# victorca25/traiNNer

Hardware: AMD Instinct MI355X
Metric: HR images/sec (G+D step), ESRGAN x4 128->512 (higher is better)
Workload: dtype f32 (bf16x3)

## Files before the change

### trainner_amd/csrc/conv_sweep.hip

```cpp
#include <stddef.h>
#include <string.h>
#include <type_traits>
#include <utility>
#include "conv_body.h"
#include "conv_epilogue.h"
#include "conv_handoff.h"

namespace {

constexpr int SW_TH = 8, SW_TW = 32, SW_HT = SW_TH + 2, SW_WT = SW_TW + 2;
constexpr int SW_ROW = TNR_X3_ROW;
constexpr int SW_A_ROWS = SW_HT * SW_WT;
constexpr int SW_A_ALLOC_ROWS = 384;
constexpr int SW_A_FLOATS = SW_A_ALLOC_ROWS * SW_ROW;
constexpr int SW_UNIT_FLOATS = 32 * SW_ROW;
constexpr int SW_SLOT_UNITS = 9;
constexpr int SW_SLOT_FLOATS = SW_SLOT_UNITS * SW_UNIT_FLOATS;
constexpr int SW_RING = 3;
constexpr size_t SW_LDS_BYTES = (size_t)(2 * SW_A_FLOATS + SW_RING * SW_SLOT_FLOATS) * sizeof(float);
constexpr int SW_NPASS = 9, SW_NSTAGE = 5, SW_NTILE = 6;
constexpr int SW_A_IT = (SW_A_ROWS * 4 + 511) / 512;
constexpr int SW_B_PIECES = (SW_SLOT_UNITS * 3 + 7) / 8;
static_assert(SW_LDS_BYTES <= 160 * 1024, "one sweep workgroup per CU");

// ... 8 lines not shown
__host__ __device__ constexpr int sw_nj_rt(int p) { return p == 7 ? 1 : ((p == 0 || p == 1 || p == 3) ? 3 : 2); }
__host__ __device__ constexpr int sw_j0_rt(int p) { return p == 0 ? 0 : (p == 2 ? 1 : (p == 4 ? 2 : (p == 5 || p == 8 ? 4 : (p == 7 ? 5 : 3)))); }
__host__ __device__ constexpr int sw_T_rt(int p) { return p == 7 ? 9 : 3; }
constexpr bool sw_plan_ok() {
    for (int p = 0; p < SW_NPASS; ++p) {
        if (SW_TT[p] * SW_NJ[p] > SW_SLOT_UNITS || 9 % SW_TT[p]) return false;
        if (sw_nj_rt(p) != SW_NJ[p] || sw_j0_rt(p) != SW_J0[p] || sw_T_rt(p) != SW_TT[p]) return false;
        if (sw_apass(p) && SW_J0[p] != (sw_phase(p) < 4 ? sw_phase(p) : 4)) return false;
        if (!sw_apass(p) && SW_J0[p] != SW_J0[p - 1] + SW_NJ[p - 1]) return false;
        if ((!sw_apass(p) || p == 8) && SW_J0[p] + SW_NJ[p] != SW_NTILE) return false;
    }
    return true;
}

static_assert(sw_plan_ok(), "sweep plan");
static_assert(SW_J0[1] == SW_J0[3] && SW_NJ[1] == SW_NJ[3] && SW_TT[1] == SW_TT[3] && SW_J0[5] == SW_J0[8] && SW_NJ[5] == SW_NJ[8] && SW_TT[5] == SW_TT[8], "passes 1 / 3 and 5 / 8 share a body");

struct SweepK {
    int nck0;
    int tiles_x, tiles_y, tpi, tiles;
    unsigned *progress;
    unsigned base;
    unsigned *err;
    int nxcd;
    unsigned *disp;
    const float *wq;
    int wq_bytes;
    ConvK st[SW_NSTAGE];
};

__host__ __device__ inline int sw_nchunks(int p, int nck0) { return sw_phase(p) == 0 ? nck0 : 2; }
__host__ __device__ inline int sw_ch_lo(int p, int nck0) { return sw_phase(p) == 0 ? 0 : 16 * nck0 + 32 * (sw_phase(p) - 1); }
__host__ __device__ inline int sw_total_units(int nck0) {
    int u = 0;
    for (int p = 0; p < SW_NPASS; ++p) u += sw_nchunks(p, nck0) * 9 * sw_nj_rt(p);
    return u;
}

struct SweepPackK {
    int nck0, units;
    int direct;
    const float *wp[SW_NSTAGE];
    int KinP[SW_NSTAGE], KoutP[SW_NSTAGE];
    float *out;
};

__device__ __forceinline__ void sweep_pack_one(const SweepPackK &a, const int g) {
    const int unit = g >> 6, r = (g >> 1) & 31, sp = g & 1;
    if (unit >= a.units) return;
    int p = 0, u0 = 0;
    for (; p < SW_NPASS; ++p) {
        const int n = sw_nchunks(p, a.nck0) * 9 * sw_nj_rt(p);
        if (unit < u0 + n) break;
        u0 += n;
    }
    const int lu = unit - u0, nj = sw_nj_rt(p);
    const int jj = lu % nj, ct = lu / nj, tap = ct % 9, ck = ct / 9;
    const int j = sw_j0_rt(p) + jj;
    const int s = j < 4 ? j : 4, cb = j == 5 ? 1 : 0;
    const int h = sp ^ ((r >> TNR_X3_SWZ) & 1);
    const int ch = sw_ch_lo(p, a.nck0) + 16 * ck + 8 * h;
    const float *src = a.wp[s] + ((size_t)tap * a.KoutP[s] + cb * 32 + r) * a.KinP[s] + ch;
    const f32x4 q0 = *reinterpret_cast<const f32x4 *>(src), q1 = *reinterpret_cast<const f32x4 *>(src + 4);
    tnr_bf16x8 pl[3];
    tnr_split_bf16x3(q0, q1, pl);
    if (a.direct) {
        float *dst = a.out + (size_t)unit * SW_UNIT_FLOATS + (h * 32 + r) * 4;
#pragma unroll
        for (int k = 0; k < 3; ++k) *reinterpret_cast<tnr_bf16x8 *>(dst + k * 256) = pl[k];
        return;
    }
    float *dst = a.out + (size_t)unit * SW_UNIT_FLOATS + r * SW_ROW + 4 * sp;
#pragma unroll
// ... 305 lines not shown
}

constexpr int S4_A_IT = (SW_A_ROWS * 4 + 255) / 256;
constexpr int S4_PIECES = (SW_SLOT_UNITS * 3 + 3) / 4;
static_assert(S4_PIECES <= 8 && S4_A_IT == 6, "the DMA / side-work plan: 8 DMA steps behind a synchronisation, 6 items per chunk");

template <int B, class F, int... I>
__device__ __forceinline__ void sw_static_for_seq(F &f, std::integer_sequence<int, I...>) {
    (f(std::integral_constant<int, B + I>{}), ...);
}
template <int B, int E, class F>
__device__ __forceinline__ void sw_static_for(F &&f) {
    sw_static_for_seq<B>(f, std::make_integer_sequence<int, (E > B ? E - B : 0)>{});
}

template <int J0, int NJ, bool DIRECT, class Sync, class Item, class Dma, class Tick, class BFetch>
__device__ __forceinline__ void sweep4_chunk(f32x16 (&acc)[2][SW_NTILE], const float *sa, const float *s_b_lane, const int (&apix0)[2],
                                             const int half, Sync &&sync, Item &&item_step, Dma &&dma_step, Tick &&tick,
                                             tnr_bf16x8 (&fbr)[3][3], BFetch &&b_fetch) {
    static_assert((9 * NJ) % 3 == 0, "a chunk starts at ring position 0");
    constexpr int TA[6] = {0, 2, 1, 0, 1, 0}, TB[6] = {2, 0, 1, 1, 0, 0};
    constexpr int NU = 9 * NJ, SU = 3 * NJ;
    tnr_bf16x8 fa[2][2][3], fb[2][3];
    const float *a_src[2][2];
    auto addr_a = [&](auto tc) __attribute__((always_inline)) {
        constexpr int t = decltype(tc)::value, dy = t / 3, dx = t % 3;
#pragma unroll
        for (int m = 0; m < 2; ++m) {
            const int pp = apix0[m] + dy * SW_WT + dx;
            a_src[t & 1][m] = sa + pp * SW_ROW + 4 * (half ^ ((pp >> TNR_X3_SWZ) & 1));
        }
    };
    auto read_a = [&](auto tc, int m, int sp) __attribute__((always_inline)) {
        constexpr int t = decltype(tc)::value;
        fa[t & 1][m][sp] = *reinterpret_cast<const tnr_bf16x8 *>(a_src[t & 1][m] + 8 * sp);
// ... 38 lines not shown
            }
            if constexpr (NEXT_TAP && i >= 3 && i < 9) read_a(std::integral_constant<int, (t + 1 < 9 ? t + 1 : 8)>{}, (i - 3) / 3, (i - 3) % 3);
            if constexpr (DMA_UNIT && i % S4_DMA_EVERY == S4_DMA_EVERY - 1) dma_step();
            if constexpr (ITEM >= 0 && ITEM < S4_A_IT && i >= 4 && i < 9) item_step(std::integral_constant<int, (ITEM >= 0 && ITEM < S4_A_IT ? ITEM : 0)>{}, std::integral_constant<int, (i >= 4 && i < 9 ? i - 4 : 0)>{});
            __builtin_amdgcn_sched_barrier(0);
        });
#ifdef SW_TIMELINE
        if constexpr (NJ == 3 || NJ == 2) {
            constexpr int cls = SYNC_UNIT ? 0 : ((u % SU) <= 1 ? 1 : (ITEM >= 0 && ITEM < S4_A_IT ? 2 : 3));
            tick(cls + (NJ == 2 ? 4 : 0), __builtin_amdgcn_s_memtime() - tu0);
        }
#endif
    });
}

template <int J0, int NJ, class Item, class BFetch>
__device__ __forceinline__ void amp4_chunk(f32x16 (&acc)[2][SW_NTILE], const float *sa, const int (&apix0)[2], const int half,
                                           Item &&item, tnr_bf16x8 (&fbq)[9], BFetch &&b_fetch) {
    constexpr int NU = 9 * NJ;
    static_assert(NU % 9 == 0, "a chunk starts at ring position 0");
    tnr_bf16x8 fa[2][2];
    const float *a_src[2][2];
    auto addr_a = [&](auto tc) __attribute__((always_inline)) {
        constexpr int t = decltype(tc)::value, dy = t / 3, dx = t % 3;
#pragma unroll
        for (int m = 0; m < 2; ++m) {
            const int pp = apix0[m] + dy * SW_WT + dx;
            a_src[t & 1][m] = sa + pp * SW_ROW + 4 * (half ^ ((pp >> TNR_X3_SWZ) & 1));
        }
    };
    addr_a(std::integral_constant<int, 0>{});
    fa[0][0] = *reinterpret_cast<const tnr_bf16x8 *>(a_src[0][0]);
// ... 9 lines not shown
        if constexpr (NEXT_TAP) fa[(t + 1) & 1][0] = *reinterpret_cast<const tnr_bf16x8 *>(a_src[(t + 1) & 1][0]);
        __builtin_amdgcn_sched_barrier(0);
        acc[1][J0 + jj] = __builtin_amdgcn_mfma_f32_32x32x16_bf16(fa[t & 1][1], fbq[u % 9], acc[1][J0 + jj], 0, 0, 0);
        if constexpr (NEXT_TAP) fa[(t + 1) & 1][1] = *reinterpret_cast<const tnr_bf16x8 *>(a_src[(t + 1) & 1][1]);
        if constexpr (ITEM >= 0 && ITEM < S4_A_IT) item(std::integral_constant<int, (ITEM >= 0 && ITEM < S4_A_IT ? ITEM : 0)>{});
        __builtin_amdgcn_sched_barrier(0);
    });
}

#ifndef S4D_EPI_AFTER
#define S4D_EPI_AFTER 1
#endif
#ifndef S4D_ALOAD_ALWAYS
#define S4D_ALOAD_ALWAYS 1
#endif
template <bool DIRECT, bool AMP = false>
__global__ void __launch_bounds__(256, 1) conv_sweep4_kernel(const SweepK c) {
    static_assert(DIRECT || !AMP, "the bf16-operand form exists as a direct form only");
    extern __shared__ __attribute__((aligned(16))) float smem[];
    float *s_a = smem, *s_b = smem + 2 * SW_A_FLOATS;
    const int tid = threadIdx.x;
    const int wave = __builtin_amdgcn_readfirstlane(tid >> 6), lane = tid & 63, li = lane & 31, half = lane >> 5;
    const int g = gridDim.x;
    const bool xcd_split = (g & 7) == 0 && c.nxcd == 8;
    const int xcd = xcd_split ? ((int)blockIdx.x & 7) : 0, per_x = xcd_split ? (g >> 3) : g;
    __shared__ int s_next_tile;
    auto next_tile = [&]() __attribute__((always_inline)) {
        if (tid == 0) {
            const int slot = (int)atomicAdd(c.disp + xcd, 1u);
            const int kk = slot / per_x, ii = slot - kk * per_x;
            s_next_tile = xcd * per_x + ii + g * kk;
        }
        __syncthreads();
// ... 92 lines not shown
                const int q = wave + 4 * i;
                if (q < pieces) __builtin_amdgcn_raw_ptr_buffer_load_lds(w_rs, dst + q * 256, 16, lane * 16, src0 + q * 1024, 0, 0);
            }
        };
        auto cur_advance = [&](SweepCur &cu) __attribute__((always_inline)) {
            cu.unit += 3 * sw_nj_rt(cu.p);
            if (++cu.sl == 3) {
                cu.sl = 0;
                if (++cu.ck == sw_nchunks(cu.p, c.nck0)) {
                    cu.ck = 0;
                    ++cu.p;
                }
            }
        };

        f32x16 acc[2][SW_NTILE];
#pragma unroll
        for (int m = 0; m < 2; ++m)
#pragma unroll
            for (int j = 0; j < SW_NTILE; ++j)
#pragma unroll
                for (int r = 0; r < 16; ++r) acc[m][j][r] = 0.f;

        SweepCur ld{0, 0, 0, 0};
        a_load(0);
        __syncthreads();
        tnr_bf16x8 fbr[3][3];
        int bq = 0;
        auto b_fetch = [&](auto rc, int sp) __attribute__((always_inline)) {
            constexpr int r = decltype(rc)::value;
            fbr[r][sp] = __builtin_bit_cast(tnr_bf16x8, __builtin_amdgcn_raw_buffer_load_b128(w_rs, lane * 16, (bq * 3 + sp) * 1024, 0));
            if (sp == 2) ++bq;
        };
        tnr_bf16x8 fbq[9];
        auto b_fetch1 = [&](auto rc) __attribute__((always_inline)) {
// ... 97 lines not shown
                conv_epilogue_dpp<TNR_CONV_3x3, SW_TW, 2, 2, true, 8>(a, t, 0, n, ty0, tx0, 0, wave, li, half, y_rs);
            }
            pend_tile = tile;
            pend_value = c.base + (unsigned)S + 1u;
            pend_age = 0;
            { SW_T(t_e1); SW_ADD(8, t_e1 - t_e0); }
        };
        auto sync = [&](auto sc) __attribute__((always_inline)) {
            constexpr int sl = decltype(sc)::value;
            slot_sync((sl + 1) % SW_RING);
        };
        auto item_step = [&](auto ic, auto kc) __attribute__((always_inline)) {
            if (has_next) item_step_buf(ic, kc, (e + 1) & 1);
        };

        sw_static_for<0, SW_NPASS>([&](auto pc) __attribute__((always_inline)) {
            constexpr int p = decltype(pc)::value;
            const int nchunks = sw_nchunks(p, c.nck0), ch_lo = sw_ch_lo(p, c.nck0);
#pragma unroll 1
            for (int ck = 0; ck < nchunks; ++ck) {
                slot_sync(1);
                if constexpr (!sw_apass(p) && !(DIRECT && S4D_EPI_AFTER)) {
                    if (ck == 0) epilogue_of(std::integral_constant<int, sw_phase(p)>{});
                }
                const bool last_ck = ck + 1 == nchunks;
                has_next = !(last_ck && p == SW_NPASS - 1);
                int ch_keep = 0;
                if (has_next) {
                    int ch_next = ch_lo + 16 * (ck + 1);
                    if (last_ck) {
                        ch_next = sw_ch_lo(p + 1 < SW_NPASS ? p + 1 : p, c.nck0);
                        if constexpr (p + 1 < SW_NPASS && sw_apass(p + 1)) {
                            const ChainWait w{c.progress, c.base + (unsigned)sw_phase(p + 1), n, ty, tx, c.tiles_x, c.tiles_y, c.err,
                                              &pend_tile, pend_value};
                            SW_T(t_w0);
                            w();
                            { SW_T(t_w1); SW_ADD(1, t_w1 - t_w0); }
                        }
                    }
                    if constexpr (!(DIRECT && S4D_ALOAD_ALWAYS)) {
                        SW_T(t_al0);
                        a_load(ch_next);
                        { SW_T(t_al1); SW_ADD(2, t_al1 - t_al0); }
                    } else {
                        ch_keep = ch_next;
                    }
                }
                if constexpr (DIRECT && S4D_ALOAD_ALWAYS) {
                    SW_T(t_al0);
                    a_load(ch_keep, has_next);
                    { SW_T(t_al1); SW_ADD(2, t_al1 - t_al0); }
                }
                const float *sa = s_a + (e & 1) * SW_A_FLOATS;
                SW_T(t_c0);
                if constexpr (AMP) {
                    auto item1 = [&](auto ic) __attribute__((always_inline)) {
                        if (has_next) a_item1(ic, (e + 1) & 1);
                    };
                    amp4_chunk<sw_j0(p), sw_nj(p)>(acc, sa, apix0, half, item1, fbq, b_fetch1);
                } else {
                    sweep4_chunk<sw_j0(p), sw_nj(p), DIRECT>(acc, sa, s_b_lane, apix0, half, sync, item_step, dma_step, tick, fbr, b_fetch);
                }
                { SW_T(t_c1); SW_ADD(6, t_c1 - t_c0); SW_ADD(15, 1ull); SW_ADD(9 + (sw_nj(p) == 3 ? 0 : (sw_nj(p) == 2 ? 1 : 2)), t_c1 - t_c0); }
                ++e;
            }
            if constexpr (DIRECT && S4D_EPI_AFTER && sw_apass(p) && p + 1 < SW_NPASS) {
                epilogue_of(std::integral_constant<int, sw_phase(p)>{});
            }
        });
        epilogue_of(std::integral_constant<int, 4>{});
    }
    asm volatile("s_waitcnt vmcnt(0)" ::: "memory");
    __syncthreads();
    if (pend_tile >= 0 && tid == 0) __hip_atomic_store(c.progress + pend_tile, pend_value, __ATOMIC_RELAXED, __HIP_MEMORY_SCOPE_AGENT);
    if (tid == 0 && atomicAdd(c.disp + 8, 1u) == (unsigned)g - 1u) {
#pragma unroll
        for (int i = 0; i < 9; ++i) __hip_atomic_store(c.disp + i, 0u, __ATOMIC_RELAXED, __HIP_MEMORY_SCOPE_AGENT);
    }
#ifdef SW_TIMELINE
    if (tid == 0) {
        tl[14] = __builtin_amdgcn_s_memtime() - tl_begin;
        for (int i = 0; i < 16; ++i) atomicAdd(&sw_tl[i], tl[i]);
        for (int i = 0; i < 16; ++i) atomicAdd(&sw_tl2[i], tl2[i]);
    }
#endif
// ... 416 lines not shown

bool d4_ok(const tnr_conv_desc *d) {
    if (d->shuffle != 0 && !(d->shuffle == 2 && (d->Cout % 256) == 0 && d->r1.ptr == nullptr && d->r2.ptr == nullptr && d->m.ptr == nullptr &&
                             d->noise_pos == 0 && d->pad_mode == 0 && (d->y.ctot % 4) == 0 &&
                             (int64_t)d->N * d->H * d->W * 4 * d->y.ctot < (1LL << 30)))
        return false;
    return d->mode == TNR_CONV_3x3 && (d->mma == TNR_MMA_BF16X3 || d->mma == TNR_MMA_BF16) && (d->pad_mode == 0 || (d->pad_mode == 1 && d->H >= 2 && d->W >= 2)) &&
           (d->Cout % 64) == 0 && d->KoutP == d->Cout &&
           d->Cin == d->KinP && (d->Cin % 16) == 0 && d->Cin >= 32 && d->Ho == d->H && d->Wo == d->W && d->W >= 32 && d->H >= 8 &&
           (int64_t)d->N * d->H * d->W * d->x.ctot < (1LL << 30) && (int64_t)d->N * d->H * d->W * d->y.ctot < (1LL << 30) &&
           (int64_t)(d->Cout / 64) * (d->Cin / 16) * 18 * SW_UNIT_FLOATS * (int64_t)sizeof(float) < (1LL << 31);
}

bool sweep_pattern(const tnr_conv_desc *st, int n, const char **why) {
    auto no = [&](const char *w) { if (why) *why = w; return false; };
    if (n != SW_NSTAGE) return no("not 5 stages");
    const tnr_conv_desc &d0 = st[0];
    if (d0.Cin < 32 || (d0.Cin % 16) != 0) return no("block input channels must be a multiple of 16, >= 32");
    for (int i = 0; i < n; ++i) {
        const tnr_conv_desc &d = st[i];
        if (d.mode != TNR_CONV_3x3 || (d.mma != TNR_MMA_BF16X3 && d.mma != TNR_MMA_BF16) || d.mma != d0.mma || d.pad_mode != 0)
            return no("stage is not a zero-padded 3x3 in bf16x3 (or all stages with bf16 operands)");
        if (d.N != d0.N || d.H != d0.H || d.W != d0.W || d.Ho != d0.H || d.Wo != d0.W) return no("pixel grids differ");
        if (d.x.ptr != d0.x.ptr || d.x.ctot != d0.x.ctot || d.x.coff != d0.x.coff) return no("stages read different buffers");
        if (d.Cin != d0.Cin + 32 * i || d.KinP != d.Cin) return no("input channels do not grow by 32 per stage");
        if (d.Cout != (i < 4 ? 32 : 64) || d.KoutP != d.Cout) return no("output channels are not 32, 32, 32, 32, 64");
        if (i < 4 && (d.y.ptr != d0.x.ptr || d.y.ctot != d0.x.ctot || d.y.coff != d0.x.coff + d.Cin)) return no("stage output is not the next channel group");
        if ((d.x.ctot % 4) || (d.x.coff % 4) || (d.y.ctot % 4) || (d.y.coff % 4)) return no("views must be 4-channel aligned");
        if (d.r1.ptr && ((d.r1.ctot % 4) || (d.r1.coff % 4) || (d.r1_ch % 4))) return no("r1 view");
        if (d.r2.ptr && ((d.r2.ctot % 4) || (d.r2.coff % 4))) return no("r2 view");
        if (d.m.ptr && ((d.m.ctot % 4) || (d.m.coff % 4) || (d.m_lo % 4) || (d.m_hi % 4))) return no("mask view");
        if (d.noise_pos < 0 || d.noise_pos > 2 || (i < 4 && d.noise_pos != 0)) return no("the noise multiplier belongs to the last stage");
        if ((int64_t)d.N * d.H * d.W * d.x.ctot >= (1LL << 30) || (int64_t)d.N * d.H * d.W * d.y.ctot >= (1LL << 30)) return no("buffer above 4 GiB");
        if (!d.x.ptr || !d.y.ptr || !d.wp) return no("null pointer");
    }
    const tnr_conv_desc &dl = st[n - 1];
    if (dl.y.ptr == d0.x.ptr && dl.y.coff < d0.x.coff + dl.Cin && dl.y.coff + dl.Cout > d0.x.coff) return no("last stage overwrites its own input");
    return true;
}

int sweep_form() {
    static const int form = [] {
        const char *w = getenv("TNR_SWEEP_WAVES"), *f = getenv("TNR_SWEEP_FORM");
        if (w && atoi(w) == 8) return 8;
        return (f && f[0] == 'd' && f[1] == 'm') ? 4 : 5;
    }();
    return form;
}
constexpr size_t S4D_LDS_BYTES = (size_t)(2 * SW_A_FLOATS) * sizeof(float);

int sweep_cus() {
    static int cus = 0;
    if (cus == 0) {
        int dev = 0;
        if (hipGetDevice(&dev) != hipSuccess || hipDeviceGetAttribute(&cus, hipDeviceAttributeMultiprocessorCount, dev) != hipSuccess ||
            hipFuncSetAttribute(reinterpret_cast<const void *>(conv_sweep_kernel), hipFuncAttributeMaxDynamicSharedMemorySize,
                                (int)SW_LDS_BYTES) != hipSuccess ||
            hipFuncSetAttribute(reinterpret_cast<const void *>(conv_sweep4_kernel<false>), hipFuncAttributeMaxDynamicSharedMemorySize,
                                (int)SW_LDS_BYTES) != hipSuccess ||
            hipFuncSetAttribute(reinterpret_cast<const void *>(conv_sweep4_kernel<true>), hipFuncAttributeMaxDynamicSharedMemorySize,
                                (int)S4D_LDS_BYTES) != hipSuccess ||
            hipFuncSetAttribute(reinterpret_cast<const void *>(conv_sweep4_kernel<true, true>), hipFuncAttributeMaxDynamicSharedMemorySize,
                                (int)S4D_LDS_BYTES) != hipSuccess || cus < 1)
            cus = -1;
    }
    return cus;
}

}

#ifdef SW_TIMELINE
extern "C" int tnr_debug_sweep_units(unsigned long long *out16, int reset) {
    if (out16 != nullptr && hipMemcpyFromSymbol(out16, HIP_SYMBOL(sw_tl2), sizeof(sw_tl2)) != hipSuccess) return TNR_ELAUNCH;
    if (reset) {
        unsigned long long z[16] = {0, 0, 0, 0, 0, 0, 0, 0, 0, 0, 0, 0, 0, 0, 0, 0};
        if (hipMemcpyToSymbol(HIP_SYMBOL(sw_tl2), z, sizeof(z)) != hipSuccess) return TNR_ELAUNCH;
    }
    return TNR_OK;
}
extern "C" int tnr_debug_sweep_timeline(unsigned long long *out16, int reset) {
    if (out16 != nullptr && hipMemcpyFromSymbol(out16, HIP_SYMBOL(sw_tl), sizeof(sw_tl)) != hipSuccess) return TNR_ELAUNCH;
    if (reset) {
        unsigned long long z[16] = {0, 0, 0, 0, 0, 0, 0, 0, 0, 0, 0, 0, 0, 0, 0, 0};
        if (hipMemcpyToSymbol(HIP_SYMBOL(sw_tl), z, sizeof(z)) != hipSuccess) return TNR_ELAUNCH;
    }
    return TNR_OK;
}
#endif

extern "C" int64_t tnr_conv_sweep_image_bytes(const tnr_conv_desc *stages, int32_t n) {
    if (stages == nullptr || !sweep_pattern(stages, n, nullptr)) return 0;
    if (stages[0].mma == TNR_MMA_BF16 && sweep_form() != 5) return 0;
    const int cus = sweep_cus();
    const int tpi = tnr_cdiv(stages[0].W, SW_TW) * tnr_cdiv(stages[0].H, SW_TH);
    if (cus < 1 || tpi > cus) return 0;
    return (int64_t)sw_total_units(stages[0].Cin / 16) * SW_UNIT_FLOATS * (int64_t)sizeof(float);
}

extern "C" int tnr_conv_sweep_pack(const tnr_conv_desc *stages, int32_t n, void *image, int64_t image_bytes, void *stream) {
    const char *why = "";
    TNR_REQUIRE(stages != nullptr && image != nullptr && sweep_pattern(stages, n, &why), "conv_sweep_pack: not a sweepable dense block (%s)", why);
    SweepPackK a;
    a.nck0 = stages[0].Cin / 16;
    a.units = sw_total_units(a.nck0);
    a.direct = sweep_form() == 5;
    TNR_REQUIRE((int64_t)a.units * SW_UNIT_FLOATS * (int64_t)sizeof(float) <= image_bytes, "conv_sweep_pack: image buffer too small");
    for (int i = 0; i < SW_NSTAGE; ++i) {
        a.wp[i] = stages[i].wp;
        a.KinP[i] = stages[i].KinP;
        a.KoutP[i] = stages[i].KoutP;
    }
    a.out = static_cast<float *>(image);
    hipLaunchKernelGGL(sweep_pack_kernel, dim3((unsigned)tnr_cdiv(a.units * 64, 256)), dim3(256), 0, (hipStream_t)stream, a);
    return tnr_check_launch("conv_sweep_pack");
}

static_assert(sizeof(SweepPackK) <= sizeof(((tnr_sweep_pack_item *)nullptr)->opaque), "tnr_sweep_pack_item holds the pack kernel's arguments");

extern "C" int tnr_conv_sweep_pack_item(const tnr_conv_desc *stages, int32_t n, void *image, int64_t image_bytes, tnr_sweep_pack_item *item) {
    const char *why = "";
    TNR_REQUIRE(stages != nullptr && image != nullptr && item != nullptr && sweep_pattern(stages, n, &why),
                "conv_sweep_pack_item: not a sweepable dense block (%s)", why);
    SweepPackK a;
    a.nck0 = stages[0].Cin / 16;
    a.units = sw_total_units(a.nck0);
    a.direct = sweep_form() == 5;
    TNR_REQUIRE((int64_t)a.units * SW_UNIT_FLOATS * (int64_t)sizeof(float) <= image_bytes, "conv_sweep_pack_item: image buffer too small");
    for (int i = 0; i < SW_NSTAGE; ++i) {
        a.wp[i] = stages[i].wp;
        a.KinP[i] = stages[i].KinP;
        a.KoutP[i] = stages[i].KoutP;
    }
    a.out = static_cast<float *>(image);
    memset(item, 0, sizeof(*item));
    memcpy(item->opaque, &a, sizeof(a));
    item->units = a.units;
    return TNR_OK;
}

extern "C" int tnr_conv_sweep_pack_batch(const tnr_sweep_pack_item *items_dev, int32_t n, int32_t max_units, void *stream) {
    TNR_REQUIRE(items_dev != nullptr && n >= 1 && n <= 65535 && max_units >= 1, "conv_sweep_pack_batch: bad arguments");
    static_assert(sizeof(tnr_sweep_pack_item) % 8 == 0, "table stride");
    hipLaunchKernelGGL(sweep_pack_batch_strided_kernel, dim3((unsigned)tnr_cdiv(max_units * 64, 256), (unsigned)n), dim3(256), 0, (hipStream_t)stream, items_dev);
    return tnr_check_launch("conv_sweep_pack_batch");
}

// ... 8 lines not shown
    TNR_REQUIRE(cus >= 1, "conv_sweep: cannot set up the kernel");
    SweepK c;
    c.nck0 = d0.Cin / 16;
    c.tiles_x = tnr_cdiv(d0.W, SW_TW);
    c.tiles_y = tnr_cdiv(d0.H, SW_TH);
    c.tpi = c.tiles_x * c.tiles_y;
    c.tiles = c.tpi * d0.N;
    TNR_REQUIRE(c.tpi <= cus, "conv_sweep: the %d tiles of an image exceed the %d co-resident workgroups", c.tpi, cus);
    c.progress = ws;
    c.err = tnr_fault_word_or(ws + ws_bytes / 4 - 1);
    static const int nxcd = [] { const char *e = getenv("TNR_SWEEP_DISPENSERS"); return e ? atoi(e) : 1; }();
    c.nxcd = nxcd == 1 ? 1 : 8;
    c.disp = ws + (ws_bytes / 4 - 1 - 4 - CH_CU_KEYS - CH_SWEEP_WORDS);
    c.base = epoch * (uint32_t)(TNR_CHAIN_MAX + 2);
    c.wq = static_cast<const float *>(image);
    c.wq_bytes = sw_total_units(c.nck0) * SW_UNIT_FLOATS * (int)sizeof(float);
    for (int i = 0; i < SW_NSTAGE; ++i) {
        const tnr_conv_desc *d = &stages[i];
        ConvK &k = c.st[i];
        k.x = d->x.ptr; k.x_ct = d->x.ctot; k.x_co = d->x.coff;
        k.N = d->N; k.H = d->H; k.W = d->W; k.Cin = d->Cin;
        k.wp = d->wp; k.KinP = d->KinP; k.KoutP = d->KoutP;
        k.y = d->y.ptr; k.y_ct = d->y.ctot; k.y_co = d->y.coff; k.Ho = d->Ho; k.Wo = d->Wo; k.Cout = d->Cout;
        k.bias = d->bias; k.act = d->act; k.slope = d->slope; k.alpha = d->alpha;
        k.r1 = d->r1.ptr; k.r1_ct = d->r1.ctot; k.r1_co = d->r1.coff; k.r1_ch = d->r1_ch; k.beta1 = d->beta1;
        k.r2 = d->r2.ptr; k.r2_ct = d->r2.ctot; k.r2_co = d->r2.coff; k.alpha2 = d->alpha2;
        k.m = d->m.ptr; k.m_ct = d->m.ctot; k.m_co = d->m.coff; k.m_lo = d->m_lo; k.m_hi = d->m_hi; k.m_slope = d->m_slope;
        k.noise_pos = d->noise_pos; k.noise_sigma = d->noise_sigma; k.noise_k0 = d->noise_key0; k.noise_k1 = d->noise_key1; k.noise_pix0 = d->noise_pix0;
        k.tiles_x = c.tiles_x; k.tiles_y = c.tiles_y; k.ncb = d->KoutP / 32;
        k.th_space = d->Ho; k.tw_space = d->Wo;
        k.ksplit = 1; k.split_stride = 0; k.bf = d->mma; k.reflect = 0;
    }
    const int per_round = (cus / c.tpi) * c.tpi;
    const int grid = c.tiles < per_round ? c.tiles : per_round;
    const int form = sweep_form();
    if (stages[0].mma == TNR_MMA_BF16) {
        TNR_REQUIRE(form == 5, "conv_sweep: bf16 operands (use_amp) run in the direct four-wave form only");
        hipLaunchKernelGGL((conv_sweep4_kernel<true, true>), dim3((unsigned)grid), dim3(256), S4D_LDS_BYTES, (hipStream_t)stream, c);
        return tnr_check_launch("conv_sweep");
    }
    if (form == 8) hipLaunchKernelGGL(conv_sweep_kernel, dim3((unsigned)grid), dim3(512), SW_LDS_BYTES, (hipStream_t)stream, c);
    else if (form == 4) hipLaunchKernelGGL(conv_sweep4_kernel<false>, dim3((unsigned)grid), dim3(256), SW_LDS_BYTES, (hipStream_t)stream, c);
    else hipLaunchKernelGGL(conv_sweep4_kernel<true>, dim3((unsigned)grid), dim3(256), S4D_LDS_BYTES, (hipStream_t)stream, c);
    return tnr_check_launch("conv_sweep");
}

extern "C" int64_t tnr_conv_wq_bytes(const tnr_conv_desc *d) {
    if (d != nullptr && s2_ok(d)) return (int64_t)(d->Cout / 64) * (d->Cin / 16) * 4 * S2_NU * SW_UNIT_FLOATS * (int64_t)sizeof(float);
    if (d == nullptr || !d4_ok(d)) return 0;
    return (int64_t)(d->Cout / 64) * (d->Cin / 16) * 18 * SW_UNIT_FLOATS * (int64_t)sizeof(float);
// ... 129 lines not shown
```

### trainner_amd/models/modules/architectures/RRDBNet_arch.py

```python
import math

import torch
import torch.nn as nn

from .... import ops
from ....engine import ConvOp, HipNet
from ....ops import View, new_act
from . import block as B


class ResidualDenseBlock_5C(nn.Module):
    def __init__(self, nf=64, gc=32, act_type="leakyrelu"):
        super().__init__()
        self.conv1 = B.conv_block(nf, gc, 3, act_type=act_type)
        self.conv2 = B.conv_block(nf + gc, gc, 3, act_type=act_type)
        self.conv3 = B.conv_block(nf + 2 * gc, gc, 3, act_type=act_type)
        self.conv4 = B.conv_block(nf + 3 * gc, gc, 3, act_type=act_type)
        self.conv5 = B.conv_block(nf + 4 * gc, nf, 3, act_type=None)


class RRDB(nn.Module):
    def __init__(self, nf, gc=32, act_type="leakyrelu"):
        super().__init__()
        self.RDB1 = ResidualDenseBlock_5C(nf, gc, act_type)
# ... 78 lines not shown
        for i in range(nrdb):
            buf = bufs[i % nbuf]
            convs = o["rdb"][i]
            st = []
            for k in range(4):
                cin = nf + gc * k
                st.append(convs[k].fwd_stage(View(buf, 0, cin), View(buf, cin, gc), fresh_from=(cin - gc if k else None),
                                             act=act, slope=sl))
            dst = View(bufs[(i + 1) % nbuf], 0, nf) if i + 1 < nrdb else View(trunk)
            nk = dict(noise=nz[i]) if nz else {}
            if i % 3 == 2:
                st.append(convs[4].fwd_stage(View(buf), dst, fresh_from=nf + 3 * gc, alpha=0.2, r1=View(buf, 0, nf),
                                             r2=View(bufs[(i - 2) % nbuf], 0, nf), alpha2=0.2, **nk))
            else:
                st.append(convs[4].fwd_stage(View(buf), dst, fresh_from=nf + 3 * gc, alpha=0.2, r1=View(buf, 0, nf), **nk))
            ops.conv_chain(st)
        y0 = new_act(N, h, w, nf, dev)
        o["lr"].fwd(View(trunk), View(y0), r1=fea_keep)
        cur, stages = View(y0), []
        for u in o["up"]:
            H2, W2 = cur.H * 2, cur.W * 2
            if self.upsample_mode == "upconv":
                nxt = View(new_act(N, H2, W2, nf, dev))
                u.fwd(cur, nxt, act=act, slope=sl)
                stages.append((cur, nxt, None))
            else:
                nxt = View(new_act(N, H2, W2, nf, dev))
                t = None
                if not u.fwd_shuffle2(cur, nxt, act=act, slope=sl):
                    t = View(new_act(N, cur.H, cur.W, 4 * nf, dev))
                    u.fwd(cur, t, act=act, slope=sl)
# ... 38 lines not shown

    def _rdb_backward(self, convs, dense, buf, GP, s, gnext, extra, want_w, pend, nz_out=None):
        nf, gc, sl = self.nf, self.gc, self.slope
        dp = self._dense_packer
        st = []
        for t in range(4):
            cin = nf + t * gc
            xk = View(buf, nf + (3 - t) * gc, gc)
            st.append(dict(x=View(GP, 0, cin), wp=dp.get(dense[t]), y=View(GP, cin, gc), fresh_from=(cin - gc if t else None),
                           mask=xk, m_lo=0, m_hi=gc, m_slope=sl))
        g = View(GP, 0, nf)
        kw = dict(r2=extra, alpha2=1.0) if extra is not None else {}
        if nz_out is not None:
            kw["noise"] = nz_out.at(2)
        st.append(dict(x=View(GP), wp=dp.get(dense[4]), y=gnext, fresh_from=nf + 3 * gc, r1=g, beta1=s, **kw))
        ops.conv_chain(st)
        if want_w:
            pend.setdefault("c5", []).append(convs[4].wgrad_item(View(buf), g, alpha=0.2 * s))
            if ops.WGRAD_PAIR and gc == 32 and nf == 64:
                for ka, kb in ((3, 2), (1, 0)):
                    cin = nf + gc * kb
                    gpair = View(GP, nf + (3 - ka) * gc, 2 * gc)
                    it = convs[ka].wgrad_item(View(buf, 0, cin), gpair)
                    it["pair"] = (convs[kb].mod.weight.grad, None if it["db"] is None else convs[kb].mod.bias.grad, gc)
                    pend["c5"].append(it)
                    ga = View(GP, nf + (3 - ka) * gc, gc)
                    pend.setdefault(gc, []).append(convs[ka].wgrad_item(View(buf, cin, gc), ga, cin_begin=cin))
                return
            for k in (3, 2, 1, 0):
                cin = nf + gc * k
                gk = View(GP, nf + (3 - k) * gc, gc)
# ... 106 lines not shown
```

### trainner_amd/ops.py

```python
import ctypes as C

import os

import torch

from . import hip
from .hip import (ACT_LRELU, ACT_NONE, ACT_RELU, CONV_1x1, CONV_3x3, CONV_3x3_C4, CONV_3x3_UP2, CONV_4x4_S2, CONV_7x7_C4, DGRAD_4x4_S2,
                  PACK_C4_DGRAD3, PACK_C4_FWD, PACK_COL_DGRAD3, PACK_COL_FWD, PACK_DENSE_DGRAD, PACK_DGRAD_3x3, PACK_DGRAD_S2, PACK_FWD, PACK_FWD_S2D, CView,
                  ConvDesc,
                  DensePackItem, PackItem, WgradDesc)


def round_up(a, b):
    return (a + b - 1) // b * b


class View:
    __slots__ = ("buf", "coff", "C")

    def __init__(self, buf, coff=0, C=None):
        assert buf.dim() == 4 and buf.dtype == torch.float32 and buf.is_contiguous()
        self.buf, self.coff = buf, coff
        self.C = buf.shape[3] - coff if C is None else C
        assert 0 <= coff and coff + self.C <= buf.shape[3]
# ... 120 lines not shown
    def add_block(self, weights, nf, gc, scale5):
        lib = hip.load()
        idx = []
        for t in range(5):
            ko, ki, n = hip.c_i(), hip.c_i(), hip.c_l()
            hip.check(lib.tnr_pack_dense_dims(nf, gc, t, C.byref(ko), C.byref(ki), C.byref(n)), "pack_dense_dims")
            self.jobs.append((list(weights), t, nf, gc, float(scale5), ko.value, ki.value, n.value))
            self.packed.append(None)
            idx.append(len(self.jobs) - 1)
        self.table = None
        return idx

    def _finalize(self):
        self.__dict__.pop("_sweep_images", None)
        self.__dict__.pop("_sweep_batch", None)
        total = sum(round_up(j[7], 64) for j in self.jobs)
        self.flat = torch.empty(total, dtype=torch.float32, device=self.device)
        items = (DensePackItem * len(self.jobs))()
        off = 0
        for i, (ws, t, nf, gc, sc, ko, ki, n) in enumerate(self.jobs):
            seg = self.flat[off:off + n]
            off += round_up(n, 64)
            it = DensePackItem()
            for k in range(5):
                it.w[k] = ws[k].data_ptr()
            it.wp, it.nf, it.gc, it.t, it.KoutP, it.KinP, it.scale5, it.n_out = seg.data_ptr(), nf, gc, t, ko, ki, sc, n
            items[i] = it
            self.packed[i] = Packed(seg, ko, ki, PACK_DENSE_DGRAD, self)
            self.max_out = max(self.max_out, n)
        self.table = torch.frombuffer(bytearray(bytes(items)), dtype=torch.uint8).to(self.device)
# ... 363 lines not shown
        if any(v[3] for v in rows):
            SWEEP_AUTO_STATE["choice"] = "layers" if any(v[0] and v[3] for v in rows) else "sweep"
    if SWEEP_AUTO_STATE["choice"] is not None:
        import logging
        logging.getLogger("base").info("dense-block form: %s (this rank: sweep %s us, per-layer %s us%s)", SWEEP_AUTO_STATE["choice"],
                                       SWEEP_AUTO_STATE["sweep_us"], SWEEP_AUTO_STATE["layers_us"],
                                       "; ranks: %s" % SWEEP_AUTO_STATE["per_rank"] if "per_rank" in SWEEP_AUTO_STATE else "")
    return SWEEP_AUTO_STATE


def conv_chain(stages):
    n = len(stages)
    assert 1 <= n <= CHAIN_MAX
    eligible = all(st.get("mode", CONV_3x3) == CONV_3x3 and st["y"].C % 32 == 0 and st["wp"].KoutP == st["y"].C for st in stages)
    crowded = COLLECTIVES_IN_FLIGHT and not CHAIN_WITH_COLLECTIVES
    sweep_ok = CONV_SWEEP and n == 5 and ((MMA == hip.MMA_BF16X3 and CHAIN_X3) or (MMA == hip.MMA_BF16 and AMP_SWEEP))
    auto = SWEEP_AUTO and CONV_CHAIN and eligible and sweep_ok and MMA == hip.MMA_BF16X3 and stages[0]["x"].buf.is_cuda
    if auto and SWEEP_AUTO_STATE["choice"] == "layers":
        for st in stages:
            conv(wino=False, **{k: v for k, v in st.items() if k != "fresh_from"})
        return
    if not CONV_CHAIN or not eligible or (crowded and not (sweep_ok and SWEEP_DISPENSED)):
        if crowded and CONV_CHAIN and eligible:
            COUNTERS["per_layer_next_to_collectives"] += 1
        for st in stages:
            conv(wino=False, **{k: v for k, v in st.items() if k != "fresh_from"})
        return
    lib = hip.load()
    descs = (ConvDesc * n)()
    fresh = (C.c_int32 * n)()
    flops = 0.0
# ... 7 lines not shown
        flops += 2.0 * st["y"].pixels * 9 * min(st["x"].C, st["wp"].KinP) * st["y"].C
    dev = stages[0]["x"].buf.device
    fault_word(dev)
    need = lib.tnr_conv_chain_workspace_bytes(C.byref(descs[0]))
    key = ("chain", str(dev), hip.stream(), need)
    ws = WS.bufs.get(key)
    if ws is None:
        ws = torch.zeros(need // 4, dtype=torch.int32, device=dev)
        WS.bufs[key] = ws
        _chain_epoch[key] = 0
    _chain_epoch[key] += 1
    if _chain_epoch[key] > 0x0FFFFFF0:
        fill(ws[:-1].view(torch.float32), 0.0)
        _chain_epoch[key] = 1
    image = None
    if CONV_SWEEP and n == 5 and (descs[0].mma == hip.MMA_BF16X3 or (descs[0].mma == hip.MMA_BF16 and AMP_SWEEP)):
        image = _sweep_image(lib, descs, n, stages, dev)
    if crowded and image is None:
        COUNTERS["per_layer_next_to_collectives"] += 1
        for st in stages:
            conv(wino=False, **{k: v for k, v in st.items() if k != "fresh_from"})
        return
    if COLLECTIVES_IN_FLIGHT:
        COUNTERS["one_launch_next_to_collectives"] += 1
    t0 = PROFILE.begin() if PROFILE is not None else None
    if image is not None:
        hip.check(lib.tnr_conv_sweep(descs, n, image.data_ptr(), ws.data_ptr(), ws.numel() * 4, _chain_epoch[key], hip.stream()), "conv_sweep")
    else:
        hip.check(lib.tnr_conv_chain(descs, fresh, n, ws.data_ptr(), ws.numel() * 4, _chain_epoch[key], hip.stream()), "conv_chain")
    if PROFILE is not None:
        x0, yl = stages[0]["x"], stages[-1]["y"]
        PROFILE.end("conv_chain", flops, t0, (x0.C, yl.C, yl.H, stages[0]["wp"].kind))


_FAULT = None


def fault_word(device=None):
    global _FAULT
    if _FAULT is None:
        _FAULT = torch.zeros(1, dtype=torch.int32, device=device if device is not None else hip.engine_device())
        hip.check(hip.load().tnr_set_fault_word(_FAULT.data_ptr()), "set_fault_word")
    return _FAULT


def chain_error_flag():
    bad = 0 if _FAULT is None else int(_FAULT.item() != 0)
# ... 473 lines not shown
```

Baseline: 74.53.

## Split dense block into four-stage sweep plus separate Winograd fifth conv

After: 76.15, median of 6. 2.2% higher.

```diff
diff --git a/trainner_amd/csrc/conv_sweep.hip b/trainner_amd/csrc/conv_sweep.hip
--- a/trainner_amd/csrc/conv_sweep.hip
+++ b/trainner_amd/csrc/conv_sweep.hip
@@ -46,6 +46,36 @@
 }
 
 static_assert(sw_plan_ok(), "sweep plan");
+
+constexpr int SW4_NPASS = 7, SW4_NSTAGE = 4, SW4_NTILE = 4;
+constexpr int SW4_J0[SW4_NPASS] =             { 0, 2, 1, 3, 2, 3, 3 };
+constexpr int SW4_NJ[SW4_NPASS] =             { 2, 2, 2, 1, 1, 1, 1 };
+__host__ __device__ constexpr int sw4_nj_rt(int p) { return p < 3 ? 2 : 1; }
+__host__ __device__ constexpr int sw4_j0_rt(int p) { return p == 0 ? 0 : (p == 2 ? 1 : ((p == 1 || p == 4) ? 2 : 3)); }
+constexpr bool sw4_plan_ok() {
+    for (int p = 0; p < SW4_NPASS; ++p) {
+        if (sw4_nj_rt(p) != SW4_NJ[p] || sw4_j0_rt(p) != SW4_J0[p]) return false;
+        if (sw_apass(p) && SW4_J0[p] != sw_phase(p)) return false;
+        if (!sw_apass(p) && SW4_J0[p] != SW4_J0[p - 1] + SW4_NJ[p - 1]) return false;
+        if ((!sw_apass(p) || p == SW4_NPASS - 1) && SW4_J0[p] + SW4_NJ[p] != SW4_NTILE) return false;
+    }
+    return true;
+}
+static_assert(sw4_plan_ok(), "four-stage sweep plan");
+
+struct SwPlan5 {
+    static constexpr int NPASS = SW_NPASS, NSTAGE = SW_NSTAGE, NTILE = SW_NTILE;
+    static constexpr int j0(int p) { return SW_J0[p]; }
+    static constexpr int nj(int p) { return SW_NJ[p]; }
+};
+struct SwPlan4 {
+    static constexpr int NPASS = SW4_NPASS, NSTAGE = SW4_NSTAGE, NTILE = SW4_NTILE;
+    static constexpr int j0(int p) { return SW4_J0[p]; }
+    static constexpr int nj(int p) { return SW4_NJ[p]; }
+};
+__host__ __device__ constexpr int sw_npass_rt(int ns) { return ns == 4 ? SW4_NPASS : SW_NPASS; }
+__host__ __device__ constexpr int sw_nj_rt(int p, int ns) { return ns == 4 ? sw4_nj_rt(p) : sw_nj_rt(p); }
+__host__ __device__ constexpr int sw_j0_rt(int p, int ns) { return ns == 4 ? sw4_j0_rt(p) : sw_j0_rt(p); }
 static_assert(SW_J0[1] == SW_J0[3] && SW_NJ[1] == SW_NJ[3] && SW_TT[1] == SW_TT[3] && SW_J0[5] == SW_J0[8] && SW_NJ[5] == SW_NJ[8] && SW_TT[5] == SW_TT[8], "passes 1 / 3 and 5 / 8 share a body");
 
 struct SweepK {
@@ -63,15 +93,16 @@
 
 __host__ __device__ inline int sw_nchunks(int p, int nck0) { return sw_phase(p) == 0 ? nck0 : 2; }
 __host__ __device__ inline int sw_ch_lo(int p, int nck0) { return sw_phase(p) == 0 ? 0 : 16 * nck0 + 32 * (sw_phase(p) - 1); }
-__host__ __device__ inline int sw_total_units(int nck0) {
+__host__ __device__ inline int sw_total_units(int nck0, int ns = SW_NSTAGE) {
     int u = 0;
-    for (int p = 0; p < SW_NPASS; ++p) u += sw_nchunks(p, nck0) * 9 * sw_nj_rt(p);
+    for (int p = 0; p < sw_npass_rt(ns); ++p) u += sw_nchunks(p, nck0) * 9 * sw_nj_rt(p, ns);
     return u;
 }
 
 struct SweepPackK {
     int nck0, units;
     int direct;
+    int ns;
     const float *wp[SW_NSTAGE];
     int KinP[SW_NSTAGE], KoutP[SW_NSTAGE];
     float *out;
@@ -81,14 +112,14 @@
     const int unit = g >> 6, r = (g >> 1) & 31, sp = g & 1;
     if (unit >= a.units) return;
     int p = 0, u0 = 0;
-    for (; p < SW_NPASS; ++p) {
-        const int n = sw_nchunks(p, a.nck0) * 9 * sw_nj_rt(p);
+    for (; p < sw_npass_rt(a.ns); ++p) {
+        const int n = sw_nchunks(p, a.nck0) * 9 * sw_nj_rt(p, a.ns);
         if (unit < u0 + n) break;
         u0 += n;
     }
-    const int lu = unit - u0, nj = sw_nj_rt(p);
+    const int lu = unit - u0, nj = sw_nj_rt(p, a.ns);
     const int jj = lu % nj, ct = lu / nj, tap = ct % 9, ck = ct / 9;
-    const int j = sw_j0_rt(p) + jj;
+    const int j = sw_j0_rt(p, a.ns) + jj;
     const int s = j < 4 ? j : 4, cb = j == 5 ? 1 : 0;
     const int h = sp ^ ((r >> TNR_X3_SWZ) & 1);
     const int ch = sw_ch_lo(p, a.nck0) + 16 * ck + 8 * h;
@@ -424,11 +455,12 @@
     sw_static_for_seq<B>(f, std::make_integer_sequence<int, (E > B ? E - B : 0)>{});
 }
 
-template <int J0, int NJ, bool DIRECT, class Sync, class Item, class Dma, class Tick, class BFetch>
-__device__ __forceinline__ void sweep4_chunk(f32x16 (&acc)[2][SW_NTILE], const float *sa, const float *s_b_lane, const int (&apix0)[2],
+template <int J0, int NJ, bool DIRECT, int NT, class Sync, class Item, class Dma, class Tick, class BFetch>
+__device__ __forceinline__ void sweep4_chunk(f32x16 (&acc)[2][NT], const float *sa, const float *s_b_lane, const int (&apix0)[2],
                                              const int half, Sync &&sync, Item &&item_step, Dma &&dma_step, Tick &&tick,
                                              tnr_bf16x8 (&fbr)[3][3], BFetch &&b_fetch) {
     static_assert((9 * NJ) % 3 == 0, "a chunk starts at ring position 0");
+    static_assert(J0 >= 0 && J0 + NJ <= NT, "the chunk's N-tiles are accumulators of the kernel");
     constexpr int TA[6] = {0, 2, 1, 0, 1, 0}, TB[6] = {2, 0, 1, 1, 0, 0};
     constexpr int NU = 9 * NJ, SU = 3 * NJ;
     tnr_bf16x8 fa[2][2][3], fb[2][3];
@@ -497,8 +529,8 @@
     });
 }
 
-template <int J0, int NJ, class Item, class BFetch>
-__device__ __forceinline__ void amp4_chunk(f32x16 (&acc)[2][SW_NTILE], const float *sa, const int (&apix0)[2], const int half,
+template <int J0, int NJ, int NT, class Item, class BFetch>
+__device__ __forceinline__ void amp4_chunk(f32x16 (&acc)[2][NT], const float *sa, const int (&apix0)[2], const int half,
                                            Item &&item, tnr_bf16x8 (&fbq)[9], BFetch &&b_fetch) {
     constexpr int NU = 9 * NJ;
     static_assert(NU % 9 == 0, "a chunk starts at ring position 0");
@@ -538,9 +570,10 @@
 #ifndef S4D_ALOAD_ALWAYS
 #define S4D_ALOAD_ALWAYS 1
 #endif
-template <bool DIRECT, bool AMP = false>
+template <bool DIRECT, bool AMP = false, class P = SwPlan5>
 __global__ void __launch_bounds__(256, 1) conv_sweep4_kernel(const SweepK c) {
     static_assert(DIRECT || !AMP, "the bf16-operand form exists as a direct form only");
+    static_assert(std::is_same<P, SwPlan5>::value || (DIRECT && !AMP), "the four-stage plan exists in the direct bf16x3 form only");
     extern __shared__ __attribute__((aligned(16))) float smem[];
     float *s_a = smem, *s_b = smem + 2 * SW_A_FLOATS;
     const int tid = threadIdx.x;
@@ -663,11 +696,11 @@
             }
         };
 
-        f32x16 acc[2][SW_NTILE];
+        f32x16 acc[2][P::NTILE];
 #pragma unroll
         for (int m = 0; m < 2; ++m)
 #pragma unroll
-            for (int j = 0; j < SW_NTILE; ++j)
+            for (int j = 0; j < P::NTILE; ++j)
 #pragma unroll
                 for (int r = 0; r < 16; ++r) acc[m][j][r] = 0.f;
 
@@ -795,7 +828,7 @@
             if (has_next) item_step_buf(ic, kc, (e + 1) & 1);
         };
 
-        sw_static_for<0, SW_NPASS>([&](auto pc) __attribute__((always_inline)) {
+        sw_static_for<0, P::NPASS>([&](auto pc) __attribute__((always_inline)) {
             constexpr int p = decltype(pc)::value;
             const int nchunks = sw_nchunks(p, c.nck0), ch_lo = sw_ch_lo(p, c.nck0);
 #pragma unroll 1
@@ -805,13 +838,13 @@
                     if (ck == 0) epilogue_of(std::integral_constant<int, sw_phase(p)>{});
                 }
                 const bool last_ck = ck + 1 == nchunks;
-                has_next = !(last_ck && p == SW_NPASS - 1);
+                has_next = !(last_ck && p == P::NPASS - 1);
                 int ch_keep = 0;
                 if (has_next) {
                     int ch_next = ch_lo + 16 * (ck + 1);
                     if (last_ck) {
-                        ch_next = sw_ch_lo(p + 1 < SW_NPASS ? p + 1 : p, c.nck0);
-                        if constexpr (p + 1 < SW_NPASS && sw_apass(p + 1)) {
+                        ch_next = sw_ch_lo(p + 1 < P::NPASS ? p + 1 : p, c.nck0);
+                        if constexpr (p + 1 < P::NPASS && sw_apass(p + 1)) {
                             const ChainWait w{c.progress, c.base + (unsigned)sw_phase(p + 1), n, ty, tx, c.tiles_x, c.tiles_y, c.err,
                                               &pend_tile, pend_value};
                             SW_T(t_w0);
@@ -838,18 +871,18 @@
                     auto item1 = [&](auto ic) __attribute__((always_inline)) {
                         if (has_next) a_item1(ic, (e + 1) & 1);
                     };
-                    amp4_chunk<sw_j0(p), sw_nj(p)>(acc, sa, apix0, half, item1, fbq, b_fetch1);
+                    amp4_chunk<P::j0(p), P::nj(p)>(acc, sa, apix0, half, item1, fbq, b_fetch1);
                 } else {
-                    sweep4_chunk<sw_j0(p), sw_nj(p), DIRECT>(acc, sa, s_b_lane, apix0, half, sync, item_step, dma_step, tick, fbr, b_fetch);
+                    sweep4_chunk<P::j0(p), P::nj(p), DIRECT>(acc, sa, s_b_lane, apix0, half, sync, item_step, dma_step, tick, fbr, b_fetch);
                 }
-                { SW_T(t_c1); SW_ADD(6, t_c1 - t_c0); SW_ADD(15, 1ull); SW_ADD(9 + (sw_nj(p) == 3 ? 0 : (sw_nj(p) == 2 ? 1 : 2)), t_c1 - t_c0); }
+                { SW_T(t_c1); SW_ADD(6, t_c1 - t_c0); SW_ADD(15, 1ull); SW_ADD(9 + (P::nj(p) == 3 ? 0 : (P::nj(p) == 2 ? 1 : 2)), t_c1 - t_c0); }
                 ++e;
             }
-            if constexpr (DIRECT && S4D_EPI_AFTER && sw_apass(p) && p + 1 < SW_NPASS) {
+            if constexpr (DIRECT && S4D_EPI_AFTER && sw_apass(p) && p + 1 < P::NPASS) {
                 epilogue_of(std::integral_constant<int, sw_phase(p)>{});
             }
         });
-        epilogue_of(std::integral_constant<int, 4>{});
+        epilogue_of(std::integral_constant<int, P::NSTAGE - 1>{});
     }
     asm volatile("s_waitcnt vmcnt(0)" ::: "memory");
     __syncthreads();
@@ -1296,7 +1329,8 @@
 
 bool sweep_pattern(const tnr_conv_desc *st, int n, const char **why) {
     auto no = [&](const char *w) { if (why) *why = w; return false; };
-    if (n != SW_NSTAGE) return no("not 5 stages");
+    if (st == nullptr || (n != SW_NSTAGE && n != SW4_NSTAGE)) return no("not 5 (or 4) stages");
+    if (n == SW4_NSTAGE && st[0].mma != TNR_MMA_BF16X3) return no("the four-stage form exists in bf16x3 only");
     const tnr_conv_desc &d0 = st[0];
     if (d0.Cin < 32 || (d0.Cin % 16) != 0) return no("block input channels must be a multiple of 16, >= 32");
     for (int i = 0; i < n; ++i) {
@@ -1317,7 +1351,7 @@
         if (!d.x.ptr || !d.y.ptr || !d.wp) return no("null pointer");
     }
     const tnr_conv_desc &dl = st[n - 1];
-    if (dl.y.ptr == d0.x.ptr && dl.y.coff < d0.x.coff + dl.Cin && dl.y.coff + dl.Cout > d0.x.coff) return no("last stage overwrites its own input");
+    if (n == SW_NSTAGE && dl.y.ptr == d0.x.ptr && dl.y.coff < d0.x.coff + dl.Cin && dl.y.coff + dl.Cout > d0.x.coff) return no("last stage overwrites its own input");
     return true;
 }
 
@@ -1343,6 +1377,8 @@
             hipFuncSetAttribute(reinterpret_cast<const void *>(conv_sweep4_kernel<true>), hipFuncAttributeMaxDynamicSharedMemorySize,
                                 (int)S4D_LDS_BYTES) != hipSuccess ||
             hipFuncSetAttribute(reinterpret_cast<const void *>(conv_sweep4_kernel<true, true>), hipFuncAttributeMaxDynamicSharedMemorySize,
+                                (int)S4D_LDS_BYTES) != hipSuccess ||
+            hipFuncSetAttribute(reinterpret_cast<const void *>(conv_sweep4_kernel<true, false, SwPlan4>), hipFuncAttributeMaxDynamicSharedMemorySize,
                                 (int)S4D_LDS_BYTES) != hipSuccess || cus < 1)
             cus = -1;
     }
@@ -1372,11 +1408,11 @@
 
 extern "C" int64_t tnr_conv_sweep_image_bytes(const tnr_conv_desc *stages, int32_t n) {
     if (stages == nullptr || !sweep_pattern(stages, n, nullptr)) return 0;
-    if (stages[0].mma == TNR_MMA_BF16 && sweep_form() != 5) return 0;
+    if ((stages[0].mma == TNR_MMA_BF16 || n == SW4_NSTAGE) && sweep_form() != 5) return 0;
     const int cus = sweep_cus();
     const int tpi = tnr_cdiv(stages[0].W, SW_TW) * tnr_cdiv(stages[0].H, SW_TH);
     if (cus < 1 || tpi > cus) return 0;
-    return (int64_t)sw_total_units(stages[0].Cin / 16) * SW_UNIT_FLOATS * (int64_t)sizeof(float);
+    return (int64_t)sw_total_units(stages[0].Cin / 16, n) * SW_UNIT_FLOATS * (int64_t)sizeof(float);
 }
 
 extern "C" int tnr_conv_sweep_pack(const tnr_conv_desc *stages, int32_t n, void *image, int64_t image_bytes, void *stream) {
@@ -1384,13 +1420,16 @@
     TNR_REQUIRE(stages != nullptr && image != nullptr && sweep_pattern(stages, n, &why), "conv_sweep_pack: not a sweepable dense block (%s)", why);
     SweepPackK a;
     a.nck0 = stages[0].Cin / 16;
-    a.units = sw_total_units(a.nck0);
+    a.ns = n;
+    a.units = sw_total_units(a.nck0, n);
     a.direct = sweep_form() == 5;
     TNR_REQUIRE((int64_t)a.units * SW_UNIT_FLOATS * (int64_t)sizeof(float) <= image_bytes, "conv_sweep_pack: image buffer too small");
+    TNR_REQUIRE(n == SW_NSTAGE || a.direct, "conv_sweep_pack: four stages run in the direct four-wave form only");
     for (int i = 0; i < SW_NSTAGE; ++i) {
-        a.wp[i] = stages[i].wp;
-        a.KinP[i] = stages[i].KinP;
-        a.KoutP[i] = stages[i].KoutP;
+        const tnr_conv_desc &d = stages[i < n ? i : n - 1];
+        a.wp[i] = d.wp;
+        a.KinP[i] = d.KinP;
+        a.KoutP[i] = d.KoutP;
     }
     a.out = static_cast<float *>(image);
     hipLaunchKernelGGL(sweep_pack_kernel, dim3((unsigned)tnr_cdiv(a.units * 64, 256)), dim3(256), 0, (hipStream_t)stream, a);
@@ -1405,13 +1444,16 @@
                 "conv_sweep_pack_item: not a sweepable dense block (%s)", why);
     SweepPackK a;
     a.nck0 = stages[0].Cin / 16;
-    a.units = sw_total_units(a.nck0);
+    a.ns = n;
+    a.units = sw_total_units(a.nck0, n);
     a.direct = sweep_form() == 5;
     TNR_REQUIRE((int64_t)a.units * SW_UNIT_FLOATS * (int64_t)sizeof(float) <= image_bytes, "conv_sweep_pack_item: image buffer too small");
+    TNR_REQUIRE(n == SW_NSTAGE || a.direct, "conv_sweep_pack_item: four stages run in the direct four-wave form only");
     for (int i = 0; i < SW_NSTAGE; ++i) {
-        a.wp[i] = stages[i].wp;
-        a.KinP[i] = stages[i].KinP;
-        a.KoutP[i] = stages[i].KoutP;
+        const tnr_conv_desc &d = stages[i < n ? i : n - 1];
+        a.wp[i] = d.wp;
+        a.KinP[i] = d.KinP;
+        a.KoutP[i] = d.KoutP;
     }
     a.out = static_cast<float *>(image);
     memset(item, 0, sizeof(*item));
@@ -1450,9 +1492,9 @@
     c.disp = ws + (ws_bytes / 4 - 1 - 4 - CH_CU_KEYS - CH_SWEEP_WORDS);
     c.base = epoch * (uint32_t)(TNR_CHAIN_MAX + 2);
     c.wq = static_cast<const float *>(image);
-    c.wq_bytes = sw_total_units(c.nck0) * SW_UNIT_FLOATS * (int)sizeof(float);
+    c.wq_bytes = sw_total_units(c.nck0, n) * SW_UNIT_FLOATS * (int)sizeof(float);
     for (int i = 0; i < SW_NSTAGE; ++i) {
-        const tnr_conv_desc *d = &stages[i];
+        const tnr_conv_desc *d = &stages[i < n ? i : n - 1];
         ConvK &k = c.st[i];
         k.x = d->x.ptr; k.x_ct = d->x.ctot; k.x_co = d->x.coff;
         k.N = d->N; k.H = d->H; k.W = d->W; k.Cin = d->Cin;
@@ -1470,6 +1512,11 @@
     const int per_round = (cus / c.tpi) * c.tpi;
     const int grid = c.tiles < per_round ? c.tiles : per_round;
     const int form = sweep_form();
+    if (n == SW4_NSTAGE) {
+        TNR_REQUIRE(form == 5, "conv_sweep: four stages run in the direct four-wave form only");
+        hipLaunchKernelGGL((conv_sweep4_kernel<true, false, SwPlan4>), dim3((unsigned)grid), dim3(256), S4D_LDS_BYTES, (hipStream_t)stream, c);
+        return tnr_check_launch("conv_sweep");
+    }
     if (stages[0].mma == TNR_MMA_BF16) {
         TNR_REQUIRE(form == 5, "conv_sweep: bf16 operands (use_amp) run in the direct four-wave form only");
         hipLaunchKernelGGL((conv_sweep4_kernel<true, true>), dim3((unsigned)grid), dim3(256), S4D_LDS_BYTES, (hipStream_t)stream, c);
diff --git a/trainner_amd/models/modules/architectures/RRDBNet_arch.py b/trainner_amd/models/modules/architectures/RRDBNet_arch.py
--- a/trainner_amd/models/modules/architectures/RRDBNet_arch.py
+++ b/trainner_amd/models/modules/architectures/RRDBNet_arch.py
@@ -116,7 +116,7 @@
                                              r2=View(bufs[(i - 2) % nbuf], 0, nf), alpha2=0.2, **nk))
             else:
                 st.append(convs[4].fwd_stage(View(buf), dst, fresh_from=nf + 3 * gc, alpha=0.2, r1=View(buf, 0, nf), **nk))
-            ops.conv_chain(st)
+            ops.dense_block(st)
         y0 = new_act(N, h, w, nf, dev)
         o["lr"].fwd(View(trunk), View(y0), r1=fea_keep)
         cur, stages = View(y0), []
@@ -185,7 +185,7 @@
         if nz_out is not None:
             kw["noise"] = nz_out.at(2)
         st.append(dict(x=View(GP), wp=dp.get(dense[4]), y=gnext, fresh_from=nf + 3 * gc, r1=g, beta1=s, **kw))
-        ops.conv_chain(st)
+        ops.dense_block(st)
         if want_w:
             pend.setdefault("c5", []).append(convs[4].wgrad_item(View(buf), g, alpha=0.2 * s))
             if ops.WGRAD_PAIR and gc == 32 and nf == 64:
diff --git a/trainner_amd/ops.py b/trainner_amd/ops.py
--- a/trainner_amd/ops.py
+++ b/trainner_amd/ops.py
@@ -158,6 +158,7 @@
     def _finalize(self):
         self.__dict__.pop("_sweep_images", None)
         self.__dict__.pop("_sweep_batch", None)
+        self.__dict__.pop("_wq_images", None)
         total = sum(round_up(j[7], 64) for j in self.jobs)
         self.flat = torch.empty(total, dtype=torch.float32, device=self.device)
         items = (DensePackItem * len(self.jobs))()
@@ -551,7 +552,7 @@
     assert 1 <= n <= CHAIN_MAX
     eligible = all(st.get("mode", CONV_3x3) == CONV_3x3 and st["y"].C % 32 == 0 and st["wp"].KoutP == st["y"].C for st in stages)
     crowded = COLLECTIVES_IN_FLIGHT and not CHAIN_WITH_COLLECTIVES
-    sweep_ok = CONV_SWEEP and n == 5 and ((MMA == hip.MMA_BF16X3 and CHAIN_X3) or (MMA == hip.MMA_BF16 and AMP_SWEEP))
+    sweep_ok = CONV_SWEEP and ((n in (4, 5) and MMA == hip.MMA_BF16X3 and CHAIN_X3) or (n == 5 and MMA == hip.MMA_BF16 and AMP_SWEEP))
     auto = SWEEP_AUTO and CONV_CHAIN and eligible and sweep_ok and MMA == hip.MMA_BF16X3 and stages[0]["x"].buf.is_cuda
     if auto and SWEEP_AUTO_STATE["choice"] == "layers":
         for st in stages:
@@ -589,7 +590,7 @@
         fill(ws[:-1].view(torch.float32), 0.0)
         _chain_epoch[key] = 1
     image = None
-    if CONV_SWEEP and n == 5 and (descs[0].mma == hip.MMA_BF16X3 or (descs[0].mma == hip.MMA_BF16 and AMP_SWEEP)):
+    if CONV_SWEEP and ((n in (4, 5) and descs[0].mma == hip.MMA_BF16X3) or (n == 5 and descs[0].mma == hip.MMA_BF16 and AMP_SWEEP)):
         image = _sweep_image(lib, descs, n, stages, dev)
     if crowded and image is None:
         COUNTERS["per_layer_next_to_collectives"] += 1
@@ -606,6 +607,48 @@
     if PROFILE is not None:
         x0, yl = stages[0]["x"], stages[-1]["y"]
         PROFILE.end("conv_chain", flops, t0, (x0.C, yl.C, yl.H, stages[0]["wp"].kind))
+
+
+DENSE_SPLIT = os.environ.get("TNR_DENSE_SPLIT", "1") != "0"
+_SWEEP_FORM_DMA = os.environ.get("TNR_SWEEP_FORM", "")[:2] == "dm"
+_cu_counts = {}
+
+
+def _cus(dev):
+    n = _cu_counts.get(dev)
+    if n is None:
+        n = _cu_counts[dev] = torch.cuda.get_device_properties(dev).multi_processor_count
+    return n
+
+
+def dense_split_applies(stages):
+    if not (DENSE_SPLIT and CONV_CHAIN and CONV_SWEEP and SWEEP_DISPENSED and CHAIN_X3 and MMA == hip.MMA_BF16X3 and len(stages) == 5):
+        return False
+    x0, yl = stages[0]["x"], stages[4]["y"]
+    if not x0.buf.is_cuda or _SWEEP_FORM_DMA:
+        return False
+    if SWEEP_AUTO and SWEEP_AUTO_STATE["choice"] == "layers":
+        return False
+    if COLLECTIVES_IN_FLIGHT and not CHAIN_WITH_COLLECTIVES:
+        return False
+    if not all(st.get("mode", CONV_3x3) == CONV_3x3 and not st.get("reflect") and st["wp"].KoutP == st["y"].C and st["wp"].KinP == st["x"].C
+               for st in stages):
+        return False
+    if yl.C != 64 or any(st["y"].C != 32 for st in stages[:4]) or x0.C % 16 or x0.C < 32 or stages[4]["x"].C != x0.C + 128:
+        return False
+    return x0.H >= 8 and x0.W >= 8 and -(-x0.W // 32) * -(-x0.H // 8) <= _cus(x0.buf.device)
+
+
+def dense_block(stages):
+    if not dense_split_applies(stages):
+        return conv_chain(stages)
+    last = {k: v for k, v in stages[4].items() if k != "fresh_from"}
+    out = last["y"]
+    for v in _stage_views(last):
+        if v is not out and v.buf.data_ptr() == out.buf.data_ptr():
+            assert min(v.coff + v.C, out.coff + out.C) <= max(v.coff, out.coff), "dense_block: the output view overlaps a view the last stage reads"
+    conv_chain(stages[:4])
+    conv(wino=True, **last)
 
 
 _FAULT = None
```
